# THGLab/NewtonNet

Hardware: AMD Instinct MI355X
Metric: atom-steps/sec (energy+force) on batched MD17 aspirin (higher is better)
Workload: dtype f32; 1 GPU; MD17 aspirin batched inference, 1024 conformers x 21 atoms per GPU, fp32, energy+force, neighbor list included (BASELINE.json configs[1]); 2 independent step(s) in flight per GPU; atoms_per_gpu=21504, weights=seed0, distinct_batches=4, steps_in_flight=2, parallelism=1 independent shard(s), no data-path collective

## Files before the change

include/newtonnet_hip.h:

```cpp
#ifndef NEWTONNET_HIP_H
#define NEWTONNET_HIP_H

#include <stddef.h>
#include <stdint.h>

#ifdef __cplusplus
extern "C" {
#endif

#define NNHIP_F 128
#define NNHIP_NB 20
#define NNHIP_MAX_NB 32
#define NNHIP_MAX_LAYERS 8
#define NNHIP_MOL_STAGE_MAX 24
#define NNHIP_N_ELEMENTS 119
#define NNHIP_ENVELOPE_COSINE (-1)

enum {
  NNHIP_ACT_SILU = 0,
  NNHIP_ACT_RELU = 1,
  NNHIP_ACT_ELU = 2,
  NNHIP_ACT_LEAKY_RELU = 3,
  NNHIP_ACT_TANH = 4,
  NNHIP_ACT_SIGMOID = 5,
// ... 105 lines not shown
  size_t msg[NNHIP_MAX_LAYERS];
  size_t h12[NNHIP_MAX_LAYERS];
  size_t phi1[NNHIP_MAX_LAYERS];
  size_t phi2[NNHIP_MAX_LAYERS];
  size_t a_mid[NNHIP_MAX_LAYERS];
  size_t a_out[NNHIP_MAX_LAYERS];
  size_t f_out[NNHIP_MAX_LAYERS];
  size_t q[NNHIP_MAX_LAYERS];
  size_t a0;
  size_t e1, e2;
  size_t g_x;
  size_t g_u;
  size_t g_a;
  size_t g_f;
  size_t total;
} nnhip_ws_layout;

int nnhip_workspace_layout(int32_t n_atoms, int32_t n_edges, int32_t n_mol, int32_t n_layers, nnhip_ws_layout* out);

int nnhip_energy_forces(const nnhip_model* model, const int64_t* z, const float* pos, const float* cell,
                        const int32_t* mol_ptr,
                        const int32_t* row_ptr, const int32_t* col, const int32_t* rev, const int32_t* pid, const float* geo,
                        const int32_t* xg, const float* disp, int32_t n_atoms, int32_t n_edges,
                        int32_t n_mol, void* workspace, size_t workspace_bytes, float* energy, float* forces,
                        float* virial, float* atom_energy, float* atom_node, float* force_node,
                        const void* prepared, void* stream);

int nnhip_graph_count_pairs_z(const float* pos, const float* cell, const int64_t* batch, const int64_t* z, int32_t n_atoms,
                              int32_t n_mol, float cutoff, int32_t* mol_ptr, int32_t* row_ptr, int32_t* status,
                              int32_t* pair_ptr, int32_t* pair_scan_scratch, void* stream);
// ... 380 lines not shown
```

newtonnet_amd/csrc/common.h:

```cpp
#pragma once
#include <hip/hip_runtime.h>
#include <stdint.h>

#include "../../include/newtonnet_hip.h"

#if (defined(EDGE_ABL_SELF) || defined(EDGE_ABL_PAIR) || defined(EDGE_ABL_TABLE) || defined(EDGE_ABL_STORE) ||              \
     defined(EDGE_ABL_NO_TABLE) || defined(EDGE_ABL_HALF_TABLE) || defined(EDGE_ABL_NOTAB) || defined(EDGE_ABL_NOMJ) || defined(MLPS_ABL_NO_H) || defined(NS_ABL_NO_Q) || defined(NS_ABL_HOT_W) || defined(MLPS_ABL_X) || defined(ABL_NO_SILU) || defined(ABL_NO_STORE) ||                  \
     (defined(LIN_ABLATE_NO_LOAD) && LIN_ABLATE_NO_LOAD) || (defined(LIN_ABLATE_NO_STORE) && LIN_ABLATE_NO_STORE) ||         \
     (defined(LIN_ABLATE_NO_MFMA) && LIN_ABLATE_NO_MFMA) || (defined(LIN_ABLATE_NO_LDS) && LIN_ABLATE_NO_LDS)) &&            \
    !defined(NNHIP_TOOLING)
#error "ablation switches produce wrong results: build through csrc/build.sh (it marks the library with -DNNHIP_TOOLING)"
#endif

#define NF NNHIP_F
#define NB NNHIP_NB
#define WAVE 64
#ifndef FT_G
#define FT_G 3072
#endif
#define FT_ROWS (FT_G + 8)
#define FT_ZERO_ROW (FT_G + 3)
#define FT_PLANE ((size_t)FT_ROWS * NNHIP_F)

typedef float f32x16 __attribute__((ext_vector_type(16)));
// ... 219 lines not shown
  float* H;
  float* Y;
  int M, ldx, ldh, ldy;
  const float* b1;
  const float* b2;
  int act;
  int h_frag;
  float* T;
  const float* T2;
  const float* Hd;
  float* G;
  const char* W1_img;
  const char* W2_img;
  int bf16;
  const int* M_dev;
};
__device__ __forceinline__ int mlp_rows(const MlpArgs& a) { return a.M_dev ? min(a.M, *a.M_dev) : a.M; }
struct MlpPair {
  MlpArgs a[2];
  int n;
  int accum[2];
};
int launch_mlp(int mode, bool accum, const MlpArgs& a, hipStream_t s);
int launch_mlp_pair(int mode, const MlpArgs& a0, bool accum0, const MlpArgs& a1, bool accum1, hipStream_t s);
bool mlp_regw_serves(int mode, const MlpPair& P);
int launch_mlp_regw(int mode, const MlpPair& P, hipStream_t s);

struct NodeFwdArgs {
  const float* f;
  const float* a_mid;
  const float* Wu;
  float* q;
  float* a_out;
  const float *W0, *b0, *W2, *b2;
  float *hn, *m;
  int N;
  int act;
};
struct NodeBwdArgs {
  const float* g_top;
  const float* h_top;
// ... 86 lines not shown
```

newtonnet_amd/csrc/edge.hip:

```cpp
#include <stdlib.h>

#include <type_traits>

#include "common.h"

#include "edge_common.h"
#include "switches.h"

template <int WPR>
__global__ void __launch_bounds__(64 * EDGE_ROWS)
msg_fwd_kernel(const float* __restrict__ m, const int2* __restrict__ xg, const float* __restrict__ table,
               const int* __restrict__ row_ptr, const int* __restrict__ col, const int* __restrict__ pid,
               const float* __restrict__ a_in, float* __restrict__ msg , float* __restrict__ a_mid,
               int n_atoms) {
  __shared__ float4 comb[EDGE_COMB_SIZE(WPR, 1)];
  int part;
  const int i_ = wave_row_split<WPR>(gridDim.x, part);
  const bool active = i_ < n_atoms;
  if (WPR == 1 && !active) return;
  const int i = active ? i_ : 0;
  const int lane = threadIdx.x & 63;
  const int c4 = 4 * (lane & 31);
  const bool hi = lane >= 32;
  const float4 mi = ld4(m + (size_t)i * NF + c4);
  float4 acc = make_float4(0.f, 0.f, 0.f, 0.f);
  const int beg = active ? row_ptr[i] : 0, end = active ? row_ptr[i + 1] : 0;
  for (int e = beg + 2 * part; e < end; e += 2 * WPR) {
    const int e1 = min(e + 1, end - 1);
    const int j0 = col[e], j1 = col[e1];
// ... 3 lines not shown
    if (!hi || e + 1 < end) {
      const FilterW fw = filter_weights(__int_as_float(gx.y));
#ifdef EDGE_ABL_HALF_TABLE
      const float4 eps = jj > i ? filter_value(table, ABL_G(gx.x), c4, fw) : mi;
#elif defined(EDGE_ABL_NOTAB)
      const float4 eps = mul4(mi, fw.w[0] + fw.w[1] + fw.w[2] + fw.w[3]);
#else
      const float4 eps = filter_value(table, ABL_G(gx.x), c4, fw);
#endif
#ifdef EDGE_ABL_NOMJ
      const float4 mj = mi;
#else
      const float4 mj = ld4(m + (size_t)ABL_J(jj, i) * NF + c4);
#endif
      const float4 v = mul4(mul4(eps, mi), mj);
      if (ABL_ST(jj > i)) {
        const int p0 = pid[e], p1 = pid[e1];
        if (EDGE_NT_MSG)
          st4_nt(msg + (size_t)(hi ? p1 : p0) * NF + c4, v);
        else
          st4(msg + (size_t)(hi ? p1 : p0) * NF + c4, v);
      }
      acc = add4(acc, v);
    }
  }
  acc = add4(acc, upper_half(acc));
  {
    float4 a1[1] = {acc};
    row_combine<WPR, 1>(a1, comb, part, lane);
    acc = a1[0];
  }
  if (active && part == 0 && !hi) st4(a_mid + (size_t)i * NF + c4, add4(ld4(a_in + (size_t)i * NF + c4), acc));
}

template <bool HAS_F, int WPR>
__global__ void __launch_bounds__(64 * EDGE_ROWS)
// ... 761 lines not shown
static bool force_fwd_mol_on() { return switches().force_fwd_mol != 0; }
static bool msg_bwd_mol_on() { return switches().msg_bwd_mol != 0; }
static bool force_direct_mol_on() { return switches().force_direct_mol != 0; }
static bool head_out_mol_on() { return switches().head_out_mol != 0; }
static bool msg_bwd_force_tail_on() { return switches().msg_bwd_force != 0 && msg_bwd_mol_on() && force_direct_mol_on(); }

void edge_config(int* small_atoms, int* mol_min, int* wpr , int* mol_forms ) {
  *small_atoms = switches().edge_small_atoms;
  *mol_min = switches().mol_kernels_min;
  wpr[0] = EDGE_WPR_MSG_FWD, wpr[1] = EDGE_WPR_FORCE_FWD, wpr[2] = EDGE_WPR_FORCE_BWD, wpr[3] = EDGE_WPR_MSG_BWD;
  *mol_forms = (force_fwd_mol_on() ? 1 : 0) | (msg_bwd_mol_on() ? 2 : 0) | (force_direct_mol_on() ? 4 : 0) | (head_out_mol_on() ? 8 : 0) |
               (msg_bwd_force_tail_on() ? 16 : 0);
}

int launch_msg_fwd(const float* m, const int* xg, const float* table, const int* row_ptr, const int* col,
                   const int* pid, const float* a_in, float* msg, float* a_mid, int n_atoms, hipStream_t s) {
  ScopedTimer t0(TC_EDGE, s);
  ScopedTimer t1(TC_EDGE_FWD_MSG, s);
  EDGE_LAUNCH(msg_fwd_kernel, EDGE_WPR_MSG_FWD, m, reinterpret_cast<const int2*>(xg), table, row_ptr, col, pid, a_in, msg, a_mid, n_atoms);
  LAUNCH_CHECK();
  return 0;
}

int launch_force_fwd(bool has_f, const float* phi1, const float* phi2, const float* geo, const int* row_ptr,
                     const int* col, const int* pid, const float* f_in, float* f_out, int n_atoms, const int* xg,
                     hipStream_t s, const int* pair_ptr, const int* mol_ptr, int n_mol) {
  ScopedTimer t0(TC_EDGE, s);
  ScopedTimer t1(TC_EDGE_FWD_FORCE, s);
  if (has_f && mol_ptr && mol_kernels_pay(n_atoms, n_mol) && force_fwd_mol_on()) {
    force_fwd_mol_kernel<<<n_mol, 64 * FM_WAVES, 0, s>>>(phi1, phi2, geo, mol_ptr, row_ptr, col, pid, f_in, f_out, n_mol,
                                                        reinterpret_cast<const int2*>(xg));
    LAUNCH_CHECK();
    return 0;
  }
// ... 240 lines not shown
```

newtonnet_amd/csrc/edge_common.h:

```cpp
#pragma once
#include <type_traits>

#include "common.h"

#define ROWS_PER_BLOCK 4
#ifndef EDGE_ROWS
#define EDGE_ROWS 4
#endif

#ifndef EDGE_NT_GH
#define EDGE_NT_GH 1
#endif
#ifndef EDGE_NT_MSG
#define EDGE_NT_MSG 0
#endif
#ifndef EDGE_NT_PHI_FWD
#define EDGE_NT_PHI_FWD 0
#endif
#ifndef EDGE_NT_PHI_BWD
#define EDGE_NT_PHI_BWD 0
#endif
#ifndef EDGE_NT_GMSG
#define EDGE_NT_GMSG 0
#endif
// ... 84 lines not shown
  FilterW f;
  const float um1 = u - 1.f, um2 = u - 2.f, up1 = u + 1.f;
  f.w[0] = -u * um1 * um2 * (1.f / 6.f);
  f.w[1] = up1 * um1 * um2 * 0.5f;
  f.w[2] = -up1 * u * um2 * 0.5f;
  f.w[3] = up1 * u * um1 * (1.f / 6.f);
  const float h = 1.0f / (float)FT_G, v = 1.f - u, uu = u * u;
  f.a = h * uu * (3.f - 2.f * u);
  f.b = h * u * v * v;
  f.c = -h * uu * v;
  f.da = 6.f * u * v;
  f.db = v * (1.f - 3.f * u);
  f.dc = u * (3.f * u - 2.f);
  return f;
}
__device__ __forceinline__ float4 filter_value(const float* __restrict__ table, int g0, int c4, const FilterW& fw) {
  float4 t[4];
#pragma unroll
  for (int k = 0; k < 4; ++k) t[k] = ld4(table + (size_t)(g0 + k) * NF + c4);
  float4 eps = mul4(t[0], fw.w[0]);
#pragma unroll
  for (int k = 1; k < 4; ++k) eps = fma4(t[k], fw.w[k], eps);
  return eps;
}
__device__ __forceinline__ void filter_value_deriv(const float* __restrict__ table, int g0, int c4, const FilterW& fw,
                                                   float4& eps, float4& deps) {
  const float* __restrict__ node = table + (size_t)(g0 + 1) * NF + c4;
  const float4 t0 = ld4(node), s0 = ld4(node + FT_PLANE), d0 = ld4(node + 2 * FT_PLANE), d1 = ld4(node + 2 * FT_PLANE + NF);
  eps = fma4(d1, fw.c, fma4(d0, fw.b, fma4(s0, fw.a, t0)));
  deps = fma4(d1, fw.dc, fma4(d0, fw.db, mul4(s0, fw.da)));
}

__device__ __forceinline__ int row_mid(const int* __restrict__ col, int beg, int end, int i, int lane);
__device__ __forceinline__ int row_mid_of(const int* __restrict__ pair_ptr, const int* __restrict__ col, int beg, int end, int i,
                                          int lane, bool active) {
#ifndef EDGE_NO_PAIR_MID
  if (pair_ptr) return active ? end - (pair_ptr[i + 1] - pair_ptr[i]) : end;
#endif
// ... 12 lines not shown
```

newtonnet_amd/csrc/mlp128.hip:

```cpp
#include <stdlib.h>
#include <string.h>

#include <atomic>

#include "common.h"
#include "switches.h"

#ifndef MLP_NT_H
#define MLP_NT_H 1
#endif
#ifndef MLP_NT_HL
#define MLP_NT_HL 1
#endif
#define MW_LD 132
#define MLP_LDS_BYTES (2 * NF * MW_LD * 4)
#ifndef MLP_WAVES
#define MLP_WAVES 8
#endif
#define MLP_THREADS (64 * MLP_WAVES)

#ifndef MLP_NT_X
#define MLP_NT_X 0
#endif
template <bool NT = false>
// ... 293 lines not shown
  nnhip_set_error("launch_mlp: unsupported mode %d/%d", mode, (int)accum_last);
  return NNHIP_E_INVALID;
}

static int mlp_wide_max_tiles(bool split_silu) {
  const int env_max = switches().mlp_wide_tiles;
  return env_max >= 0 ? env_max : (split_silu ? MLPS_WIDE_MAX_TILES : MLP_WIDE_MAX_TILES);
}
int mlp_wide_max_tiles_silu() { return mlp_wide_max_tiles(split_products_enabled()); }
static bool mlp_use_wide(const MlpArgs& a) {
  return cdiv(a.M, 32) <= mlp_wide_max_tiles(split_products_enabled() && a.act == NNHIP_ACT_SILU) || a.b1 || a.b2;
}

int launch_mlp(int mode, bool accum, const MlpArgs& a, hipStream_t s) {
  if (a.M <= 0) return 0;
  ScopedTimer t0(TC_LIN, s);
  ScopedTimer t1((a.b1 || a.b2) ? TC_LIN1 : TC_MLP, s);
  if (mlp_use_wide(a)) {
    MlpArgs w = a;
    if (w.h_frag) w.ldh = NF;
    return launch_mlp_wide(mode, accum, w, s);
  }
  if (mode < MODE_FWD || mode > MODE_TAN2 || ((mode == MODE_TAN || mode == MODE_TAN2) && a.h_frag)) {
    nnhip_set_error("launch_mlp: unsupported mode %d", mode);
    return NNHIP_E_INVALID;
  }
  MlpPair P;
  P.a[0] = P.a[1] = a;
  P.n = 1;
  P.accum[0] = P.accum[1] = accum ? 1 : 0;
  if (split_products_enabled() && mlp_regw_serves(mode, P)) {
    ScopedTimer t2(TC_MLP_ONEPASS, s);
    return launch_mlp_regw(mode, P, s);
  }
  return launch_mlp_dispatch(mode, accum, P, s);
}

int launch_mlp_pair(int mode, const MlpArgs& a0, bool accum0, const MlpArgs& a1, bool accum1, hipStream_t s) {
  if (a0.M != a1.M || mode < MODE_FWD || mode > MODE_TAN2 || accum0 || a0.h_frag != a1.h_frag || a0.act != a1.act ||
      a0.ldh != a1.ldh) {
    nnhip_set_error("launch_mlp_pair: bad arguments");
    return NNHIP_E_INVALID;
  }
  if (a0.M <= 0) return 0;
  if (mlp_use_wide(a0) || mlp_use_wide(a1)) {
    if (a0.b1 || a0.b2 || a1.b1 || a1.b2 || (mode == MODE_FWD && accum1)) {
      const int rc = launch_mlp(mode, accum0, a0, s);
      return rc ? rc : launch_mlp(mode, accum1, a1, s);
    }
    ScopedTimer t0(TC_LIN, s);
    ScopedTimer t1(TC_MLP, s);
    MlpPair W;
    W.a[0] = a0;
    W.a[1] = a1;
    if (W.a[0].h_frag) W.a[0].ldh = W.a[1].ldh = NF;
    W.n = 2;
    W.accum[0] = 0;
    W.accum[1] = accum1 ? 1 : 0;
    return launch_mlp_wide_pair(mode, W, s);
// ... 108 lines not shown
```

newtonnet_amd/csrc/mlp128r.hip:

```cpp
#include <stdlib.h>

#include "common.h"
#include "switches.h"

typedef _Float16 h8 __attribute__((ext_vector_type(8)));
typedef _Float16 h4 __attribute__((ext_vector_type(4)));
typedef __bf16 b8 __attribute__((ext_vector_type(8)));
typedef __bf16 b4 __attribute__((ext_vector_type(4)));

#define RW_WAVES 8
#define RW_THREADS (64 * RW_WAVES)
#define RW_PITCH 272
#define RW_PLANE (32 * RW_PITCH)
#define RW_TILE (2 * RW_PLANE)
#define RW_WIMG_PLANE (NF * NF * 2)

struct RwLds {
  char xt[2][RW_TILE];
  char at[2][RW_TILE];
  float pmax[2][8 * 32];
  float invx[2][32];
  float4 part[2][4][4 * 64];
  unsigned bar[2];
  unsigned xbar;
// ... 163 lines not shown
#define RW_DBG() { ++dbg_k; dbg_t[dbg_k] = wall_clock64(); dbg_s[dbg_k] += dbg_t[dbg_k] - dbg_t[dbg_k - 1]; }
#define RW_DBG_PRINT()                                                                                                        \
  if (blockIdx.x == 3 && lane == 0 && (wave == 0 || wave == 5)) {                                                              \
    const double d_ = 100.0 * dbg_tiles;                                                                                      \
    printf("regw mode %d wave %d: %d tiles, us per tile: waitX %.2f commitX %.2f req+bar %.2f gemm1 %.2f epi1 %.2f bar %.2f commit+bar %.2f gemm2 %.2f epi2 %.2f\n", \
           MODE, wave, dbg_tiles, dbg_s[1] / d_, dbg_s[2] / d_, dbg_s[3] / d_, dbg_s[4] / d_, dbg_s[5] / d_, dbg_s[6] / d_, dbg_s[7] / d_,        \
           dbg_s[8] / d_, dbg_s[9] / d_);                                                                                                    \
  }
#else
#define RW_DBG_DECL()
#define RW_DBG_TOP()
#define RW_DBG()
#define RW_DBG_PRINT()
#endif

template <int MODE, bool SINGLE = false, bool SHARED_X = (MODE == MODE_FWD && !SINGLE)>
__global__ void __launch_bounds__(RW_THREADS, 2) mlp_regw_kernel(const MlpPair P) {
  constexpr bool OWN_X = !SHARED_X;
  constexpr bool TRAIN = MODE == MODE_TAN || MODE == MODE_TAN2;
  extern __shared__ __attribute__((aligned(16))) char lds_raw[];
  RwLds& L = *reinterpret_cast<RwLds*>(lds_raw);
  const int lane = threadIdx.x & 63;
  const int wave = __builtin_amdgcn_readfirstlane(threadIdx.x >> 6);
  const int g = wave >> 2, nb = wave & 3;
  const int r = lane & 31, h = lane >> 5;
  const int M = mlp_rows(P.a[0]);
  if (M <= 0) return;
  const int n_tiles = (M + 31) >> 5;
  const bool bf = TRAIN && *reinterpret_cast<const int*>(P.a[0].W1_img + 2 * RW_WIMG_PLANE + 4) == WIMG_FMT_BF16;

  const int ga = SINGLE ? 0 : g;
  RwFrag w1, w2;
// ... 11 lines not shown
  float* Tg = ga ? P.a[1].T : P.a[0].T;
  const float* T2g = ga ? P.a[1].T2 : P.a[0].T2;
  const float* Hdg = ga ? P.a[1].Hd : P.a[0].Hd;
  float* Gg = ga ? P.a[1].G : P.a[0].G;
  const int tile0 = SINGLE ? 2 * (int)blockIdx.x + g : (int)blockIdx.x;
  const int tile_step = SINGLE ? 2 * (int)gridDim.x : (int)gridDim.x;
  unsigned* bar = &L.bar[g];
  unsigned bar_target = 0, xbar_target = 0;

  if (threadIdx.x == 0) L.xbar = 0;
  if (threadIdx.x < 2) L.bar[threadIdx.x] = 0;
  if (threadIdx.x < 4) L.ready[threadIdx.x] = L.taken[threadIdx.x] = 0;
  __syncthreads();

  float4 xq[NX], hq[4];
  auto request = [&](int tile) {
    const int tc = min(tile, n_tiles - 1);
#pragma unroll
    for (int i = 0; i < NX; ++i) {
      const int row = min((tc << 5) + xrow0 + 2 * i + h, M - 1);
      xq[i] = MODE == MODE_BWD ? ld4_nt(Xg + (size_t)row * ldx + 4 * r) : ld4(Xg + (size_t)row * ldx + 4 * r);
    }
    if (MODE == MODE_BWD) {
      const float4* hp = reinterpret_cast<const float4*>(Hg) + ((size_t)tc * 4 + nb) * 256 + lane;
#pragma unroll
      for (int q = 0; q < 4; ++q) hq[q] = ld4_nt(reinterpret_cast<const float*>(hp + 64 * q));
    }
    if (TRAIN) {
      const float* hp = Hg + (size_t)min((tc << 5) + r, M - 1) * ldh + nb * 32 + 4 * h;
#pragma unroll
      for (int q = 0; q < 4; ++q) hq[q] = ld4(hp + 8 * q);
    }
  };
  request(tile0);
  RW_DBG_DECL()

  int k = 0;
  for (int tile = tile0; tile < n_tiles; tile += tile_step, ++k) {
    RW_DBG_TOP()
    const int e = (tile << 5) + r;
    const bool live = e < M;
    char* xtile = L.xt[OWN_X ? g : (k & 1)];
    float* invx = L.invx[OWN_X ? g : (k & 1)];
#ifdef RW_CLOCK_DEBUG
    asm volatile("" ::"v"(xq[NX - 1].w));
    RW_DBG()
#endif
#pragma unroll
    for (int i = 0; i < NX; ++i) {
      if (bf)
        rw_commit_row_bf(xq[i], xtile, invx, xrow0 + 2 * i + h, r);
      else
        rw_commit_row(xq[i], xtile, invx, xrow0 + 2 * i + h, r, h);
    }
    float4 hin[4];
    if (MODE != MODE_FWD) {
#pragma unroll
      for (int q = 0; q < 4; ++q) hin[q] = hq[q];
    }
    RW_DBG()
    request(tile + tile_step);
    if (!OWN_X)
      rw_group_sync(&L.xbar, xbar_target, lane, 8);
    else
      rw_group_sync(bar, bar_target, lane);
    RW_DBG()
    float a[16];
    {
// ... 47 lines not shown
      float m = 0.f;
#pragma unroll
      for (int q = 0; q < 16; ++q) m = fmaxf(m, fabsf(a[q]));
      L.pmax[g][(nb * 2 + h) * 32 + r] = m;
    }
    RW_DBG()
    rw_group_sync(bar, bar_target, lane);
    RW_DBG()
    float inv2 = 1.0f;
    if (bf)
      rw_commit_block_bf(a, L.at[g], nb, r, h);
    else
      inv2 = rw_commit_block(a, L.at[g], L.pmax[g], nb, r, h);
    rw_group_sync(bar, bar_target, lane);
    RW_DBG()
    {
      const f32x16 acc = bf ? rw_gemm_bf(L.at[g], w2, r, h) : rw_gemm(L.at[g], w2, r, h);
      RW_DBG()
      const float sc = inv2 * w2.inv;
      if (SHARED_X || SINGLE) {
        if (live) {
          float4* yp = reinterpret_cast<float4*>(Yg + (size_t)e * ldy + nb * 32 + 4 * h);
#pragma unroll
          for (int q = 0; q < 4; ++q)
            yp[2 * q] = make_float4(acc[4 * q] * sc, acc[4 * q + 1] * sc, acc[4 * q + 2] * sc, acc[4 * q + 3] * sc);
        }
      } else if (g == 1) {
        rw_spin_until(&L.taken[nb], (unsigned)(k - 1));
#pragma unroll
        for (int q = 0; q < 4; ++q)
// ... 32 lines not shown
  const int single = mlp_regw_single();
  if (mode == MODE_TAN || mode == MODE_TAN2) {
    if (level <= 0 || !switches().mlp_regw_train || P.n < 1 || P.n > 2) return false;
    for (int k = 0; k < P.n; ++k) {
      const MlpArgs& a = P.a[k];
      if (!a.W1_img || !a.W2_img || a.h_frag || a.act != NNHIP_ACT_SILU || a.b1 || a.b2 || a.M_dev || a.ldh != P.a[0].ldh) return false;
      if (mode == MODE_TAN ? !a.T : (!a.T2 || !a.Hd || !a.G)) return false;
    }
    if (P.n == 1) return !P.accum[0];
    if (mode == MODE_TAN && P.a[0].X == P.a[1].X && P.a[0].ldx == P.a[1].ldx && P.a[0].Y != P.a[1].Y && !P.accum[0] && !P.accum[1])
      return true;
    return P.a[0].Y == P.a[1].Y && P.a[0].ldy == P.a[1].ldy && !P.accum[0] && P.accum[1];
  }
  if (P.n == 1)
    return level > 0 && ((mode == MODE_BWD && single >= 1) || (mode == MODE_FWD && single >= 2)) && P.a[0].W1_img &&
           P.a[0].W2_img && P.a[0].h_frag && P.a[0].act == NNHIP_ACT_SILU && !P.a[0].b1 && !P.a[0].b2 && !P.accum[0];
  if (level <= 0 || P.n != 2 || !((mode == MODE_BWD) || (mode == MODE_FWD && level >= 2))) return false;
  for (int k = 0; k < 2; ++k)
    if (!P.a[k].W1_img || !P.a[k].W2_img || !P.a[k].h_frag || P.a[k].act != NNHIP_ACT_SILU || P.a[k].b1 || P.a[k].b2) return false;
  if (mode == MODE_FWD) return P.a[0].X == P.a[1].X && P.a[0].ldx == P.a[1].ldx && !P.accum[0] && !P.accum[1];
  return P.a[0].Y == P.a[1].Y && P.a[0].ldy == P.a[1].ldy && !P.accum[0] && P.accum[1];
}
template <int MODE, bool SINGLE, bool SHARED_X = (MODE == MODE_FWD && !SINGLE)>
static int launch_regw_t(const MlpPair& P, hipStream_t s) {
  static const hipError_t attr_rc = hipFuncSetAttribute((const void*)mlp_regw_kernel<MODE, SINGLE, SHARED_X>,
                                                        hipFuncAttributeMaxDynamicSharedMemorySize, (int)sizeof(RwLds));
  HIP_TRY(attr_rc);
  const int n_tiles = (P.a[0].M + 31) / 32;
  const int units = SINGLE ? (n_tiles + 1) / 2 : n_tiles;
  const int blocks = units < 256 ? units : 256;
  mlp_regw_kernel<MODE, SINGLE, SHARED_X><<<blocks, RW_THREADS, sizeof(RwLds), s>>>(P);
  LAUNCH_CHECK();
  return 0;
}
int launch_mlp_regw(int mode, const MlpPair& P, hipStream_t s) {
  if (mode == MODE_TAN && P.n == 2 && P.a[0].X == P.a[1].X && !P.accum[1]) return launch_regw_t<MODE_TAN, false, true>(P, s);
  if (mode == MODE_TAN) return P.n == 1 ? launch_regw_t<MODE_TAN, true>(P, s) : launch_regw_t<MODE_TAN, false>(P, s);
  if (mode == MODE_TAN2) return P.n == 1 ? launch_regw_t<MODE_TAN2, true>(P, s) : launch_regw_t<MODE_TAN2, false>(P, s);
  if (P.n == 1) return mode == MODE_FWD ? launch_regw_t<MODE_FWD, true>(P, s) : launch_regw_t<MODE_BWD, true>(P, s);
  return mode == MODE_FWD ? launch_regw_t<MODE_FWD, false>(P, s) : launch_regw_t<MODE_BWD, false>(P, s);
}
```

newtonnet_amd/csrc/pipeline.hip:

```cpp
#include <stdarg.h>
#include <stdio.h>
#include <string.h>

#include <atomic>
#include <mutex>
#include <algorithm>
#include <vector>

#include "common.h"
#include "switches.h"

int launch_filter_tables(const float* const* edge_w, float* const* tables, int n_layers, const float* freq, int nb,
                         int envelope, hipStream_t s);
int launch_msg_fwd(const float* m, const int* xg, const float* table, const int* row_ptr, const int* col,
                   const int* pid, const float* a_in, float* msg, float* a_mid, int n_atoms, hipStream_t s);
int launch_force_fwd(bool has_f, const float* phi1, const float* phi2, const float* geo, const int* row_ptr,
                     const int* col, const int* pid, const float* f_in, float* f_out, int n_atoms, const int* xg, hipStream_t s,
                     const int* pair_ptr = nullptr, const int* mol_ptr = nullptr, int n_mol = 0);
int launch_force_bwd(bool has_f, const float* gf, const float* phi1, const float* phi2, const float* geo,
                     const int* row_ptr, const int* col, const int* pid, const float* f_in, float* g_h12, float* g_u,
                     float* g_fin, int n_atoms, const int* xg, hipStream_t s, const int* pair_ptr = nullptr, const int* rev = nullptr);
int launch_msg_bwd(const float* g_msg, const float* g_a, const float* m, const int* xg, const float* table,
                   const int* row_ptr, const int* col, const int* pid, float* g_m, float* g_x, int n_atoms, bool need_gm,
                   hipStream_t s, const int* pair_ptr = nullptr, const int* mol_ptr = nullptr, int n_mol = 0,
                   const MsgBwdForceTail* tail = nullptr, bool* tail_done = nullptr);
int launch_geometry_bwd(const float* g_x, const float* g_u, const float* geo, const float* disp, const float* pos,
                        const float* cell, const int* row_ptr, const int* col, const int* rev, const int* mol_ptr,
                        int n_atoms, int n_edges, int n_mol, int n_layers, float cutoff, float* g_d, float* forces,
                        float* virial, hipStream_t s, bool small_molecules = false);
int launch_layer_norm_fwd(float* a, const float* gamma, const float* beta, int n_atoms, float* xhat, float* rstd,
// ... 49 lines not shown
    }
  };
  put("{\"version\": %d, \"tooling_build\": %d, \"split_f16_products\": %d, ", nnhip_version(), nnhip_build_flags(), forms & 1);
  put("\"neighbor_list\": {\"single_launch_max_atoms\": %d, \"per_molecule_kernels\": %d, \"cell_list\": \"one periodic molecule (host choice)\"}, ",
      nnhip_graph_small_max_atoms(), graph_mol_on() ? 1 : 0);
  put("\"edge_rows\": {\"waves_per_row\": {\"msg_fwd\": %d, \"force_fwd\": %d, \"force_bwd\": %d, \"msg_bwd\": %d}, \"four_waves_per_row_up_to_atoms\": %d}, ",
      wpr[0], wpr[1], wpr[2], wpr[3], small_atoms);
  put("\"molecule_forms\": {\"max_atoms\": %d, \"edge_kernels_from_molecules\": %d, \"force_fwd\": %d, \"msg_bwd\": %d, \"force_direct\": %d, \"head_out\": %d, "
      "\"msg_bwd_with_forces\": %d}, ",
      NNHIP_MOL_STAGE_MAX, mol_min, mol_forms & 1, (mol_forms >> 1) & 1, (mol_forms >> 2) & 1, (mol_forms >> 3) & 1, (mol_forms >> 4) & 1);
  put("\"edge_mlp\": {\"row_local_up_to_tiles\": %d, \"one_pass_adjoint\": %d, \"one_pass_forward\": %d, \"one_pass_single_adjoint\": %d, "
      "\"one_pass_single_forward\": %d}, ",
      mlp_wide_max_tiles_silu(), (forms >> 1) & 1, (forms >> 2) & 1, (forms >> 3) & 1, (forms >> 4) & 1);
  put("\"node_turn_fused\": %d, ", ((forms & 1) && node_turn_enabled()) ? 1 : 0);
  put("\"node_bwd_recomputes_q\": %d, ", ((forms & 1) && node_bwd_q_enabled()) ? 1 : 0);
  put("\"radial_table_intervals\": %d, \"env\": {", FT_G);
  bool first = true;
  for (const char* nm : names) {
    const char* v = switch_text(nm);
    if (!v) continue;
    char clean[25];
    int k = 0;
    for (; k < 24 && v[k]; ++k) {
      const char ch = v[k];
      const bool ok = (ch >= '0' && ch <= '9') || (ch >= 'a' && ch <= 'z') || (ch >= 'A' && ch <= 'Z') || ch == '_' || ch == '.' ||
                      ch == ',' || ch == '+' || ch == '-';
      clean[k] = ok ? ch : '?';
    }
    clean[k] = 0;
    put("%s\"%s\": \"%s\"", first ? "" : ", ", nm, clean);
// ... 184 lines not shown
  w.pub.e1 = carve(off, nf);
  w.pub.e2 = carve(off, nf);
  w.pub.g_x = carve(off, (size_t)L * E * 4);
  w.pub.g_u = carve(off, (size_t)L * E * 16);
  w.pub.g_a = carve(off, nf);
  w.pub.g_f = carve(off, 3 * nf);
  w.g_f2 = carve(off, 3 * nf);
  w.gf_mid = carve(off, 3 * nf);
  w.g_h12 = carve(off, 2 * ef);
  w.g_msg = carve(off, ef);
  w.g_m = carve(off, nf);
  w.g_e = carve(off, nf);
  w.g_d = carve(off, (size_t)E * 16);
  w.atom_energy = carve(off, (size_t)N * 4);
  w.prep = carve(off, prep_bytes(L));
  w.pub.total = off;
}

extern "C" size_t nnhip_workspace_bytes(int32_t N, int32_t E, int32_t B, int32_t L) {
  if (N < 0 || E < 0 || L < 1 || L > NNHIP_MAX_LAYERS) return 0;
  WsInternal w;
  make_layout(N, E, B, L, w);
  return w.pub.total;
}

extern "C" int nnhip_workspace_layout(int32_t N, int32_t E, int32_t B, int32_t L, nnhip_ws_layout* out) {
  if (!out || N < 0 || E < 0 || L < 1 || L > NNHIP_MAX_LAYERS) {
    nnhip_set_error("nnhip_workspace_layout: bad arguments");
    return NNHIP_E_INVALID;
  }
// ... 306 lines not shown

  PrepLayout pq;
  make_prep_layout(L, pq);
  char* pbase = prepared ? (char*)prepared : ws + w.prep;
  auto Q = [&](size_t off) { return (float*)(pbase + off); };
  if (!prepared) TRY(run_prepare(model, pq, pbase, s));
  const bool split_nodes = split_products_enabled() && act == NNHIP_ACT_SILU;
  if (!embedded) TRY(launch_embed(z, model->node_embedding, Q(pq.m_tab), N, P(w.pub.a0), P(w.pub.m[0]), s));
  const float* a_in = P(w.pub.a0);
  const float* f_in = nullptr;
  auto A_OUT = [&](int l) { return (l == L - 1 && atom_node_out) ? atom_node_out : P(w.pub.a_out[l]); };
  auto F_OUT = [&](int l) { return (l == L - 1 && force_node_out) ? force_node_out : P(w.pub.f_out[l]); };
  const bool node_turn = split_nodes && want_forces && !model->layer[L - 1].ln_w && node_turn_enabled();
  const bool recompute_q = split_nodes && want_forces && node_bwd_q_enabled();
  auto q_stored = [&](int l) { return want_forces && !(recompute_q && !model->layer[l].ln_w); };
  for (int l = 0; l < L; ++l) {
    const nnhip_layer_params& lp = model->layer[l];
    const bool has_f = l > 0;
    {
      TRY(launch_msg_fwd(P(w.pub.m[l]), xg, Q(pq.ftab[l]), row_ptr, col, pid, a_in, P(w.pub.msg[l]), P(w.pub.a_mid[l]), N, s));
      if (E > 0) {
        float* h12 = P(w.pub.h12[l]);
        MlpArgs m1 = {P(w.pub.msg[l]), lp.eq1_0_w, lp.eq1_2_w, h12, P(w.pub.phi1[l]), P_, NF, NF, NF};
        MlpArgs m2 = {P(w.pub.msg[l]), lp.eq2_0_w, lp.eq2_2_w, h12 + h2_off, P(w.pub.phi2[l]), P_, NF, NF, NF};
        m1.h_frag = m2.h_frag = 1;
        m1.act = m2.act = act;
        m1.M_dev = m2.M_dev = n_pairs_dev;
        if (split_nodes) {
          m1.W1_img = pbase + pq.img[l][IMG_EQ1_0];
          m1.W2_img = pbase + pq.img[l][IMG_EQ1_2];
          m2.W1_img = pbase + pq.img[l][IMG_EQ2_0];
          m2.W2_img = pbase + pq.img[l][IMG_EQ2_2];
        }
        if (has_f)
          TRY(launch_mlp_pair(MODE_FWD, m1, false, m2, false, s));
        else
          TRY(launch_mlp(MODE_FWD, false, m1, s));
      }
      TRY(launch_force_fwd(has_f, P(w.pub.phi1[l]), P(w.pub.phi2[l]), geo, row_ptr, col, pid, f_in, F_OUT(l), N, mask_xg, s, pair_ptr,
                           mol_kernels ? mol_ptr : nullptr, B));
    }
    if (!(node_turn && l == L - 1)) {
      NodeFwdArgs na;
      memset(&na, 0, sizeof(na));
      na.f = F_OUT(l);
      na.a_mid = P(w.pub.a_mid[l]);
      na.Wu = lp.update_w;
// ... 415 lines not shown
```

newtonnet_amd/csrc/switches.h:

```cpp
#pragma once
#include <stdlib.h>

#ifndef EDGE_SMALL_ATOMS
#define EDGE_SMALL_ATOMS 2048
#endif

#define NNHIP_SWITCH_TABLE(X)                                                                                                      \
  X(long, lnum, edge_lds, "NNHIP_EDGE_LDS", 0)                         \
  X(int, num, edge_small_atoms, "NNHIP_EDGE_SMALL_ATOMS", EDGE_SMALL_ATOMS)  \
  X(int, num, edge_wpr, "NNHIP_EDGE_WPR", 0)                           \
  X(int, flag, force_bwd_owner_gu, "NNHIP_FORCE_BWD_OWNER_GU", 1)      \
  X(int, flag, force_direct_mol, "NNHIP_FORCE_DIRECT_MOL", 1)          \
  X(int, flag, force_fwd_mol, "NNHIP_FORCE_FWD_MOL", 1)                \
  X(int, flag, graph_mol, "NNHIP_GRAPH_MOL", 1)                        \
  X(int, num, graph_small_atoms, "NNHIP_GRAPH_SMALL_ATOMS", 128)       \
  X(int, flag, head_out_mol, "NNHIP_HEAD_OUT_MOL", 1)                  \
  X(int, num, lin_blocks, "NNHIP_LIN_BLOCKS", 512)                     \
  X(int, num, mlp_regw, "NNHIP_MLP_REGW", 1)                           \
  X(int, num, mlp_regw_single, "NNHIP_MLP_REGW_SINGLE", 1)             \
  X(int, flag, mlp_regw_train, "NNHIP_MLP_REGW_TRAIN", 1)              \
  X(int, flag, mlp_split, "NNHIP_MLP_SPLIT", 1)                        \
  X(int, num, mlp_wide_tiles, "NNHIP_MLP_WIDE_TILES", -1)              \
  X(int, num, mol_kernels_min, "NNHIP_MOL_KERNELS_MIN", 640)           \
  X(int, flag, msg_bwd_force, "NNHIP_MSG_BWD_FORCE", 1)                \
  X(int, flag, msg_bwd_mol, "NNHIP_MSG_BWD_MOL", 1)                    \
  X(int, flag, node_bwd_q, "NNHIP_NODE_BWD_Q", 1)                      \
  X(int, flag, node_turn, "NNHIP_NODE_TURN", 1)

struct Switches {
#define X(type, kind, field, name, dflt) type field;
  NNHIP_SWITCH_TABLE(X)
#undef X
};

inline const char* const kSwitchNames[] = {
#define X(type, kind, field, name, dflt) name,
    NNHIP_SWITCH_TABLE(X)
#undef X
};
inline const char* const kPythonSwitchNames[] = {"NNHIP_TRAIN_BF16", "NNHIP_WGRAD_FORM", "NNHIP_WGRAD_RPC"};
// ... 19 lines not shown
```

Measured before the change: 15.89 million atom-steps/s.

## Form pair messages on-chip inside the paired MLP kernel instead of storing them

For layers after the first, the message kernel no longer writes the per-pair message rows (pairs x 128 floats) to global memory. Instead, layer 0 records compact per-pair records (i, j, table index, filter weight). The register-weight MLP kernel then rebuilds each message on the fly from m_i, m_j and the radial filter table, with prefetching pipelined across tiles. This removes a large write and re-read of edge-sized tensors. In exchange each MLP tile does more scattered gathers of node rows and table rows, and the path only applies when the launch meets the regw/split conditions.

```diff
diff --git a/include/newtonnet_hip.h b/include/newtonnet_hip.h
--- a/include/newtonnet_hip.h
+++ b/include/newtonnet_hip.h
@@ -143,6 +143,7 @@
   size_t g_a;
   size_t g_f;
   size_t total;
+  size_t pair_rec;
 } nnhip_ws_layout;
 
 int nnhip_workspace_layout(int32_t n_atoms, int32_t n_edges, int32_t n_mol, int32_t n_layers, nnhip_ws_layout* out);
diff --git a/newtonnet_amd/csrc/common.h b/newtonnet_amd/csrc/common.h
--- a/newtonnet_amd/csrc/common.h
+++ b/newtonnet_amd/csrc/common.h
@@ -257,6 +257,9 @@
   const char* W2_img;
   int bf16;
   const int* M_dev;
+  const int* pair_rec;
+  const float* msg_m;
+  const float* msg_table;
 };
 __device__ __forceinline__ int mlp_rows(const MlpArgs& a) { return a.M_dev ? min(a.M, *a.M_dev) : a.M; }
 struct MlpPair {
@@ -268,6 +271,8 @@
 int launch_mlp_pair(int mode, const MlpArgs& a0, bool accum0, const MlpArgs& a1, bool accum1, hipStream_t s);
 bool mlp_regw_serves(int mode, const MlpPair& P);
 int launch_mlp_regw(int mode, const MlpPair& P, hipStream_t s);
+bool mlp_msg_onchip(int M, int act, int n_atoms);
+bool mlp_msg_onchip_enabled();
 
 struct NodeFwdArgs {
   const float* f;
diff --git a/newtonnet_amd/csrc/edge.hip b/newtonnet_amd/csrc/edge.hip
--- a/newtonnet_amd/csrc/edge.hip
+++ b/newtonnet_amd/csrc/edge.hip
@@ -12,7 +12,7 @@
 msg_fwd_kernel(const float* __restrict__ m, const int2* __restrict__ xg, const float* __restrict__ table,
                const int* __restrict__ row_ptr, const int* __restrict__ col, const int* __restrict__ pid,
                const float* __restrict__ a_in, float* __restrict__ msg , float* __restrict__ a_mid,
-               int n_atoms) {
+               int n_atoms, int4* __restrict__ pair_rec ) {
   __shared__ float4 comb[EDGE_COMB_SIZE(WPR, 1)];
   int part;
   const int i_ = wave_row_split<WPR>(gridDim.x, part);
@@ -46,12 +46,16 @@
       const float4 mj = ld4(m + (size_t)ABL_J(jj, i) * NF + c4);
 #endif
       const float4 v = mul4(mul4(eps, mi), mj);
-      if (ABL_ST(jj > i)) {
+      if (jj > i && (msg || pair_rec)) {
         const int p0 = pid[e], p1 = pid[e1];
-        if (EDGE_NT_MSG)
-          st4_nt(msg + (size_t)(hi ? p1 : p0) * NF + c4, v);
-        else
-          st4(msg + (size_t)(hi ? p1 : p0) * NF + c4, v);
+        const size_t p = (size_t)(hi ? p1 : p0);
+        if (ABL_ST(msg != nullptr)) {
+          if (EDGE_NT_MSG)
+            st4_nt(msg + p * NF + c4, v);
+          else
+            st4(msg + p * NF + c4, v);
+        }
+        if (pair_rec && c4 == 0) pair_rec[p] = make_int4(i, jj, gx.x, gx.y);
       }
       acc = add4(acc, v);
     }
@@ -843,10 +847,11 @@
 }
 
 int launch_msg_fwd(const float* m, const int* xg, const float* table, const int* row_ptr, const int* col,
-                   const int* pid, const float* a_in, float* msg, float* a_mid, int n_atoms, hipStream_t s) {
+                   const int* pid, const float* a_in, float* msg, float* a_mid, int n_atoms, hipStream_t s, int* pair_rec) {
   ScopedTimer t0(TC_EDGE, s);
   ScopedTimer t1(TC_EDGE_FWD_MSG, s);
-  EDGE_LAUNCH(msg_fwd_kernel, EDGE_WPR_MSG_FWD, m, reinterpret_cast<const int2*>(xg), table, row_ptr, col, pid, a_in, msg, a_mid, n_atoms);
+  EDGE_LAUNCH(msg_fwd_kernel, EDGE_WPR_MSG_FWD, m, reinterpret_cast<const int2*>(xg), table, row_ptr, col, pid, a_in, msg, a_mid, n_atoms,
+              reinterpret_cast<int4*>(pair_rec));
   LAUNCH_CHECK();
   return 0;
 }
diff --git a/newtonnet_amd/csrc/edge_common.h b/newtonnet_amd/csrc/edge_common.h
--- a/newtonnet_amd/csrc/edge_common.h
+++ b/newtonnet_amd/csrc/edge_common.h
@@ -122,14 +122,17 @@
   f.dc = u * (3.f * u - 2.f);
   return f;
 }
+__device__ __forceinline__ float4 filter_combine(const float4 (&t)[4], const FilterW& fw) {
+  float4 eps = mul4(t[0], fw.w[0]);
+#pragma unroll
+  for (int k = 1; k < 4; ++k) eps = fma4(t[k], fw.w[k], eps);
+  return eps;
+}
 __device__ __forceinline__ float4 filter_value(const float* __restrict__ table, int g0, int c4, const FilterW& fw) {
   float4 t[4];
 #pragma unroll
   for (int k = 0; k < 4; ++k) t[k] = ld4(table + (size_t)(g0 + k) * NF + c4);
-  float4 eps = mul4(t[0], fw.w[0]);
-#pragma unroll
-  for (int k = 1; k < 4; ++k) eps = fma4(t[k], fw.w[k], eps);
-  return eps;
+  return filter_combine(t, fw);
 }
 __device__ __forceinline__ void filter_value_deriv(const float* __restrict__ table, int g0, int c4, const FilterW& fw,
                                                    float4& eps, float4& deps) {
diff --git a/newtonnet_amd/csrc/mlp128.hip b/newtonnet_amd/csrc/mlp128.hip
--- a/newtonnet_amd/csrc/mlp128.hip
+++ b/newtonnet_amd/csrc/mlp128.hip
@@ -331,6 +331,10 @@
 
 int launch_mlp(int mode, bool accum, const MlpArgs& a, hipStream_t s) {
   if (a.M <= 0) return 0;
+  if (a.pair_rec) {
+    nnhip_set_error("launch_mlp: pair records given where the launch reads stored rows");
+    return NNHIP_E_INVALID;
+  }
   ScopedTimer t0(TC_LIN, s);
   ScopedTimer t1((a.b1 || a.b2) ? TC_LIN1 : TC_MLP, s);
   if (mlp_use_wide(a)) {
@@ -360,6 +364,21 @@
     return NNHIP_E_INVALID;
   }
   if (a0.M <= 0) return 0;
+  if (a0.pair_rec || a1.pair_rec) {
+    MlpPair P;
+    P.a[0] = a0;
+    P.a[1] = a1;
+    P.n = 2;
+    P.accum[0] = P.accum[1] = 0;
+    if (accum1 || mlp_use_wide(a0) || !split_products_enabled() || !mlp_regw_serves(mode, P)) {
+      nnhip_set_error("launch_mlp_pair: pair records given where the launch reads stored rows");
+      return NNHIP_E_INVALID;
+    }
+    ScopedTimer t0(TC_LIN, s);
+    ScopedTimer t1(TC_MLP, s);
+    ScopedTimer t2(TC_MLP_ONEPASS, s);
+    return launch_mlp_regw(mode, P, s);
+  }
   if (mlp_use_wide(a0) || mlp_use_wide(a1)) {
     if (a0.b1 || a0.b2 || a1.b1 || a1.b2 || (mode == MODE_FWD && accum1)) {
       const int rc = launch_mlp(mode, accum0, a0, s);
diff --git a/newtonnet_amd/csrc/mlp128r.hip b/newtonnet_amd/csrc/mlp128r.hip
--- a/newtonnet_amd/csrc/mlp128r.hip
+++ b/newtonnet_amd/csrc/mlp128r.hip
@@ -1,6 +1,7 @@
 #include <stdlib.h>
 
 #include "common.h"
+#include "edge_common.h"
 #include "switches.h"
 
 typedef _Float16 h8 __attribute__((ext_vector_type(8)));
@@ -201,8 +202,9 @@
 #define RW_DBG_PRINT()
 #endif
 
-template <int MODE, bool SINGLE = false, bool SHARED_X = (MODE == MODE_FWD && !SINGLE)>
+template <int MODE, bool SINGLE = false, bool SHARED_X = (MODE == MODE_FWD && !SINGLE), bool MSG_ONCHIP = false>
 __global__ void __launch_bounds__(RW_THREADS, 2) mlp_regw_kernel(const MlpPair P) {
+  static_assert(!MSG_ONCHIP || (MODE == MODE_FWD && SHARED_X), "pair messages are formed in the shared-X forward only");
   constexpr bool OWN_X = !SHARED_X;
   constexpr bool TRAIN = MODE == MODE_TAN || MODE == MODE_TAN2;
   extern __shared__ __attribute__((aligned(16))) char lds_raw[];
@@ -244,7 +246,32 @@
   __syncthreads();
 
   float4 xq[NX], hq[4];
+  const int4* const rec = reinterpret_cast<const int4*>(P.a[0].pair_rec);
+  const char* const msg_m = reinterpret_cast<const char*>(P.a[0].msg_m);
+  const char* const msg_tab = reinterpret_cast<const char*>(P.a[0].msg_table);
+  int4 rq[NX];
+  float4 mq[NX][2], tq[NX][4];
+  int uq[NX];
+  auto rec_of = [&](int tile, int i) { return rec[min((min(tile, n_tiles - 1) << 5) + xrow0 + 2 * i + h, M - 1)]; };
+  auto request_ops = [&](const int4& rc, int b) {
+    mq[b][0] = *reinterpret_cast<const float4*>(msg_m + ((unsigned)rc.x * (NF * 4u) + 16u * r));
+    mq[b][1] = *reinterpret_cast<const float4*>(msg_m + ((unsigned)rc.y * (NF * 4u) + 16u * r));
+#pragma unroll
+    for (int q = 0; q < 4; ++q) tq[b][q] = *reinterpret_cast<const float4*>(msg_tab + ((unsigned)(rc.z + q) * (NF * 4u) + 16u * r));
+    uq[b] = rc.w;
+  };
+  auto formed = [&](int b) { return mul4(mul4(filter_combine(tq[b], filter_weights(__int_as_float(uq[b]))), mq[b][0]), mq[b][1]); };
+  auto request_recs = [&](int tile) {
+#pragma unroll
+    for (int i = 0; i < NX; ++i) rq[i] = rec_of(tile, i);
+  };
+  if (MSG_ONCHIP) request_recs(tile0);
   auto request = [&](int tile) {
+    if (MSG_ONCHIP) {
+#pragma unroll
+      for (int i = 0; i < NX; ++i) request_ops(rq[i], i);
+      return;
+    }
     const int tc = min(tile, n_tiles - 1);
 #pragma unroll
     for (int i = 0; i < NX; ++i) {
@@ -263,6 +290,7 @@
     }
   };
   request(tile0);
+  if (MSG_ONCHIP) request_recs(tile0 + tile_step);
   RW_DBG_DECL()
 
   int k = 0;
@@ -273,15 +301,16 @@
     char* xtile = L.xt[OWN_X ? g : (k & 1)];
     float* invx = L.invx[OWN_X ? g : (k & 1)];
 #ifdef RW_CLOCK_DEBUG
-    asm volatile("" ::"v"(xq[NX - 1].w));
+    asm volatile("" ::"v"(MSG_ONCHIP ? tq[NX - 1][3].w : xq[NX - 1].w));
     RW_DBG()
 #endif
 #pragma unroll
     for (int i = 0; i < NX; ++i) {
+      const float4 xv = MSG_ONCHIP ? formed(i) : xq[i];
       if (bf)
-        rw_commit_row_bf(xq[i], xtile, invx, xrow0 + 2 * i + h, r);
+        rw_commit_row_bf(xv, xtile, invx, xrow0 + 2 * i + h, r);
       else
-        rw_commit_row(xq[i], xtile, invx, xrow0 + 2 * i + h, r, h);
+        rw_commit_row(xv, xtile, invx, xrow0 + 2 * i + h, r, h);
     }
     float4 hin[4];
     if (MODE != MODE_FWD) {
@@ -359,6 +388,7 @@
       inv2 = rw_commit_block(a, L.at[g], L.pmax[g], nb, r, h);
     rw_group_sync(bar, bar_target, lane);
     RW_DBG()
+    if (MSG_ONCHIP) request_recs(tile + 2 * tile_step);
     {
       const f32x16 acc = bf ? rw_gemm_bf(L.at[g], w2, r, h) : rw_gemm(L.at[g], w2, r, h);
       RW_DBG()
@@ -421,22 +451,31 @@
   }
   if (P.n == 1)
     return level > 0 && ((mode == MODE_BWD && single >= 1) || (mode == MODE_FWD && single >= 2)) && P.a[0].W1_img &&
-           P.a[0].W2_img && P.a[0].h_frag && P.a[0].act == NNHIP_ACT_SILU && !P.a[0].b1 && !P.a[0].b2 && !P.accum[0];
-  if (level <= 0 || P.n != 2 || !((mode == MODE_BWD) || (mode == MODE_FWD && level >= 2))) return false;
-  for (int k = 0; k < 2; ++k)
+           P.a[0].W2_img && P.a[0].h_frag && P.a[0].act == NNHIP_ACT_SILU && !P.a[0].b1 && !P.a[0].b2 && !P.accum[0] && !P.a[0].pair_rec;
+  const bool onchip = mode == MODE_FWD && P.n == 2 && P.a[0].pair_rec && P.a[0].pair_rec == P.a[1].pair_rec && P.a[0].msg_m &&
+                      P.a[0].msg_table && !P.a[0].X && !P.a[1].X;
+  if (level <= 0 || P.n != 2 || !((mode == MODE_BWD) || (mode == MODE_FWD && (level >= 2 || onchip)))) return false;
+  for (int k = 0; k < 2; ++k) {
     if (!P.a[k].W1_img || !P.a[k].W2_img || !P.a[k].h_frag || P.a[k].act != NNHIP_ACT_SILU || P.a[k].b1 || P.a[k].b2) return false;
+    if (P.a[k].pair_rec && !onchip) return false;
+  }
   if (mode == MODE_FWD) return P.a[0].X == P.a[1].X && P.a[0].ldx == P.a[1].ldx && !P.accum[0] && !P.accum[1];
   return P.a[0].Y == P.a[1].Y && P.a[0].ldy == P.a[1].ldy && !P.accum[0] && P.accum[1];
 }
-template <int MODE, bool SINGLE, bool SHARED_X = (MODE == MODE_FWD && !SINGLE)>
+int mlp_wide_max_tiles_silu();
+bool mlp_msg_onchip_enabled() { return switches().msg_onchip && split_products_enabled() && mlp_regw_level() >= 1; }
+bool mlp_msg_onchip(int M, int act, int n_atoms) {
+  return mlp_msg_onchip_enabled() && act == NNHIP_ACT_SILU && (M + 31) / 32 > mlp_wide_max_tiles_silu() && n_atoms < (1 << 23);
+}
+template <int MODE, bool SINGLE, bool SHARED_X = (MODE == MODE_FWD && !SINGLE), bool MSG_ONCHIP = false>
 static int launch_regw_t(const MlpPair& P, hipStream_t s) {
-  static const hipError_t attr_rc = hipFuncSetAttribute((const void*)mlp_regw_kernel<MODE, SINGLE, SHARED_X>,
+  static const hipError_t attr_rc = hipFuncSetAttribute((const void*)mlp_regw_kernel<MODE, SINGLE, SHARED_X, MSG_ONCHIP>,
                                                         hipFuncAttributeMaxDynamicSharedMemorySize, (int)sizeof(RwLds));
   HIP_TRY(attr_rc);
   const int n_tiles = (P.a[0].M + 31) / 32;
   const int units = SINGLE ? (n_tiles + 1) / 2 : n_tiles;
   const int blocks = units < 256 ? units : 256;
-  mlp_regw_kernel<MODE, SINGLE, SHARED_X><<<blocks, RW_THREADS, sizeof(RwLds), s>>>(P);
+  mlp_regw_kernel<MODE, SINGLE, SHARED_X, MSG_ONCHIP><<<blocks, RW_THREADS, sizeof(RwLds), s>>>(P);
   LAUNCH_CHECK();
   return 0;
 }
@@ -445,5 +484,6 @@
   if (mode == MODE_TAN) return P.n == 1 ? launch_regw_t<MODE_TAN, true>(P, s) : launch_regw_t<MODE_TAN, false>(P, s);
   if (mode == MODE_TAN2) return P.n == 1 ? launch_regw_t<MODE_TAN2, true>(P, s) : launch_regw_t<MODE_TAN2, false>(P, s);
   if (P.n == 1) return mode == MODE_FWD ? launch_regw_t<MODE_FWD, true>(P, s) : launch_regw_t<MODE_BWD, true>(P, s);
+  if (mode == MODE_FWD && P.a[0].pair_rec) return launch_regw_t<MODE_FWD, false, true, true>(P, s);
   return mode == MODE_FWD ? launch_regw_t<MODE_FWD, false>(P, s) : launch_regw_t<MODE_BWD, false>(P, s);
 }
diff --git a/newtonnet_amd/csrc/pipeline.hip b/newtonnet_amd/csrc/pipeline.hip
--- a/newtonnet_amd/csrc/pipeline.hip
+++ b/newtonnet_amd/csrc/pipeline.hip
@@ -13,7 +13,7 @@
 int launch_filter_tables(const float* const* edge_w, float* const* tables, int n_layers, const float* freq, int nb,
                          int envelope, hipStream_t s);
 int launch_msg_fwd(const float* m, const int* xg, const float* table, const int* row_ptr, const int* col,
-                   const int* pid, const float* a_in, float* msg, float* a_mid, int n_atoms, hipStream_t s);
+                   const int* pid, const float* a_in, float* msg, float* a_mid, int n_atoms, hipStream_t s, int* pair_rec = nullptr);
 int launch_force_fwd(bool has_f, const float* phi1, const float* phi2, const float* geo, const int* row_ptr,
                      const int* col, const int* pid, const float* f_in, float* f_out, int n_atoms, const int* xg, hipStream_t s,
                      const int* pair_ptr = nullptr, const int* mol_ptr = nullptr, int n_mol = 0);
@@ -93,6 +93,7 @@
       mlp_wide_max_tiles_silu(), (forms >> 1) & 1, (forms >> 2) & 1, (forms >> 3) & 1, (forms >> 4) & 1);
   put("\"node_turn_fused\": %d, ", ((forms & 1) && node_turn_enabled()) ? 1 : 0);
   put("\"node_bwd_recomputes_q\": %d, ", ((forms & 1) && node_bwd_q_enabled()) ? 1 : 0);
+  put("\"msg_formed_on_chip\": %d, ", mlp_msg_onchip_enabled() ? 1 : 0);
   put("\"radial_table_intervals\": %d, \"env\": {", FT_G);
   bool first = true;
   for (const char* nm : names) {
@@ -307,6 +308,7 @@
   w.g_d = carve(off, (size_t)E * 16);
   w.atom_energy = carve(off, (size_t)N * 4);
   w.prep = carve(off, prep_bytes(L));
+  w.pub.pair_rec = carve(off, (size_t)((E + 1) / 2) * 16);
   w.pub.total = off;
 }
 
@@ -643,11 +645,15 @@
   const bool node_turn = split_nodes && want_forces && !model->layer[L - 1].ln_w && node_turn_enabled();
   const bool recompute_q = split_nodes && want_forces && node_bwd_q_enabled();
   auto q_stored = [&](int l) { return want_forces && !(recompute_q && !model->layer[l].ln_w); };
+  const bool onchip_layers = L > 1 && E > 0 && split_nodes && mlp_msg_onchip(P_, act, N);
   for (int l = 0; l < L; ++l) {
     const nnhip_layer_params& lp = model->layer[l];
     const bool has_f = l > 0;
     {
-      TRY(launch_msg_fwd(P(w.pub.m[l]), xg, Q(pq.ftab[l]), row_ptr, col, pid, a_in, P(w.pub.msg[l]), P(w.pub.a_mid[l]), N, s));
+      const bool onchip = has_f && onchip_layers;
+      int* const pair_rec = reinterpret_cast<int*>(ws + w.pub.pair_rec);
+      TRY(launch_msg_fwd(P(w.pub.m[l]), xg, Q(pq.ftab[l]), row_ptr, col, pid, a_in, onchip ? nullptr : P(w.pub.msg[l]), P(w.pub.a_mid[l]),
+                         N, s, (l == 0 && onchip_layers) ? pair_rec : nullptr));
       if (E > 0) {
         float* h12 = P(w.pub.h12[l]);
         MlpArgs m1 = {P(w.pub.msg[l]), lp.eq1_0_w, lp.eq1_2_w, h12, P(w.pub.phi1[l]), P_, NF, NF, NF};
@@ -660,6 +666,12 @@
           m1.W2_img = pbase + pq.img[l][IMG_EQ1_2];
           m2.W1_img = pbase + pq.img[l][IMG_EQ2_0];
           m2.W2_img = pbase + pq.img[l][IMG_EQ2_2];
+        }
+        if (onchip) {
+          m1.X = m2.X = nullptr;
+          m1.pair_rec = m2.pair_rec = pair_rec;
+          m1.msg_m = m2.msg_m = P(w.pub.m[l]);
+          m1.msg_table = m2.msg_table = Q(pq.ftab[l]);
         }
         if (has_f)
           TRY(launch_mlp_pair(MODE_FWD, m1, false, m2, false, s));
diff --git a/newtonnet_amd/csrc/switches.h b/newtonnet_amd/csrc/switches.h
--- a/newtonnet_amd/csrc/switches.h
+++ b/newtonnet_amd/csrc/switches.h
@@ -24,6 +24,7 @@
   X(int, num, mol_kernels_min, "NNHIP_MOL_KERNELS_MIN", 640)           \
   X(int, flag, msg_bwd_force, "NNHIP_MSG_BWD_FORCE", 1)                \
   X(int, flag, msg_bwd_mol, "NNHIP_MSG_BWD_MOL", 1)                    \
+  X(int, flag, msg_onchip, "NNHIP_MSG_ONCHIP", 1)                      \
   X(int, flag, node_bwd_q, "NNHIP_NODE_BWD_Q", 1)                      \
   X(int, flag, node_turn, "NNHIP_NODE_TURN", 1)
 
```

Result: no change. 15.92 million atom-steps/s (median of 2 runs) (+0.2%).
